# arhik/GaussianSplat

Hardware: AMD Instinct MI355X
Metric: fwd+bwd Msplats/sec at 1M Gaussians, 1920x1080, SH deg 3 (higher is better)
Workload: dtype f32; 1 GPU; C3: 1000000 gaussians, 1920x1080, SH3, ONE camera view per step, fwd+bwd; the steps cycle over the cameras [0, 4] (view k: eye rotated about +y by 45k degrees; one view slot per camera); synthetic scene of SURVEY 8d with the quaternions NORMALISED (8d leaves N(0,1)^4 raw: the reference never normalises q and |q| scales every footprint by |q|^4; un-normalised q is parity-tested, tests/test_gpu_size; views_per_rank=1, nranks=1, settle_steps=24, rank_mode=1, binning_rounds=1, schedule=3, view_slots=True, order=depth_desc, tile=16, instances=30150056, coarse_instances=2175944, walked_fwd=8350144, alpha_cull=True, list_cap=0, tile_parts=1, lists_capped=False

## Files before the change

gaussiansplat_amd/backend.py:

```python
from __future__ import annotations

import ctypes as C
import os

import numpy as np

_HERE = os.path.dirname(os.path.abspath(__file__))
LIB_PATH = os.environ.get("GSPLAT_HIP_LIB") or os.path.join(_HERE, "lib", "libgsplat_hip.so")

GS_MEM_HOST, GS_MEM_DEVICE = 0, 1
ORDER_INDEX, ORDER_DEPTH_DESC, ORDER_DEPTH_ASC = 0, 1, 2

(ARR_TS, ARR_TPS, ARR_MU, ARR_COV3D, ARR_COV2D, ARR_INVCOV, ARR_BBS, ARR_RGB, ARR_SIG, ARR_DEPTH_KEY,
 ARR_TILE_RECT, ARR_SORT_IDXS, ARR_TILE_RANGES, ARR_SORTED_IDS, ARR_SORTED_KEYS, ARR_GRAD2D) = range(16)

STAGES = ("preprocess", "depth_sort", "count_scan", "emit", "tile_sort", "ranges", "composite_fwd",
          "composite_bwd", "preprocess_bwd")

SYMBOLS = ("gs_default_config", "gs_abi_version", "gs_create", "gs_destroy", "gs_last_error", "gs_set_stream",
           "gs_synchronize", "gs_set_model", "gs_set_model_2d", "gs_set_image_size", "gs_set_camera", "gs_preprocess", "gs_bin", "gs_bind_outputs", "gs_forward", "gs_backward_sgd",
           "gs_backward", "gs_backward_ex", "gs_reset_grads", "gs_loss_l1_dssim", "gs_sgd_step", "gs_comm_unique_id",
           "gs_comm_init", "gs_allreduce_grads", "gs_comm_destroy", "gs_color_grads_pack", "gs_sh_grads_from_views", "gs_grads_alloc", "gs_grads_read", "gs_num_gaussians", "gs_num_instances", "gs_get_array",
           "gs_get_stage_times", "gs_get_stage_stats", "gs_get_work_counters", "gs_get_work_counters_ex", "gs_debug_time_composite",
           "gs_debug_tile_clock", "gs_debug_clock_mhz", "gs_rank_probe_result", "gs_num_rounds", "gs_set_view_slot", "gs_num_coarse_instances",
           "gs_get_list_stats", "gs_get_tile_parts", "gs_get_bin_path", "gs_debug_set_window", "gs_debug_tile_clock_rows", "gs_debug_tail_fill",
           "gs_adam_step", "gs_backward_adam")

GS_ABI_VERSION = 3
GS_DEBUG_WIDE_CURSORS = 1
GS_DEBUG_ALWAYS_ORDER = 2
GS_DEBUG_SUPER16 = 8
GS_DEBUG_SUPER8 = 16
GS_DEBUG_NO_TAIL_FILL = 32
GS_DEBUG_TINY_CAPS = 4
GS_MAX_VIEW_SLOTS = 4096
GS_ADAM_GROUPS = 6
GS_ADAM_SELECTIVE = 1
GS_ERR_INVALID, GS_ERR_UNSUPPORTED = -1, -5


class GsConfig(C.Structure):
    _fields_ = [("struct_size", C.c_int32), ("abi_version", C.c_int32), ("tile_size", C.c_int32), ("order", C.c_int32), ("t_min", C.c_float),
                ("deterministic", C.c_int32), ("export_debug", C.c_int32), ("profile_stages", C.c_int32),
                ("bin_path", C.c_int32), ("rank_mode", C.c_int32), ("alpha_cull", C.c_int32), ("schedule", C.c_int32),
                ("slab_mode", C.c_int32), ("slab_max_ratio", C.c_float), ("slab_fractions", C.c_float * 3), ("debug_flags", C.c_int32),
                ("depth_sort", C.c_int32), ("list_cap", C.c_int32), ("tile_parts", C.c_int32), ("reserved", C.c_int32 * 3)]


class GsGrads(C.Structure):
    _fields_ = [("d_means", C.c_void_p), ("d_scales", C.c_void_p), ("d_quats", C.c_void_p),
                ("d_opacities", C.c_void_p), ("d_shs", C.c_void_p)]


class GsError(RuntimeError):
    def __init__(self, code: int, msg: str):
        super().__init__(f"libgsplat_hip error {code}: {msg}")
# ... 397 lines not shown
```

gaussiansplat_amd/build.py:

```python
from __future__ import annotations

import os
import subprocess
import sys
from concurrent.futures import ThreadPoolExecutor

HERE = os.path.dirname(os.path.abspath(__file__))
CSRC = os.path.join(HERE, "csrc")
OUT_DIR = os.path.join(HERE, "lib")
LIB = os.path.join(OUT_DIR, "libgsplat_hip.so")
ARCH = "gfx950"

SOURCES = {
    "gs_preprocess.hip": ["-ffp-contract=off"],
    "gs_preprocess2d.hip": ["-ffp-contract=off"],
    "gs_preprocess_bwd.hip": [],
    "gs_sort.hip": [],
    "gs_bin2.hip": [],
    "gs_bin3.hip": [],
    "gs_bin_small.hip": [],
    "gs_composite.hip": ["-fno-slp-vectorize"],
    "gs_loss.hip": ["-fno-slp-vectorize"],
    "gs_adam.hip": ["-ffp-contract=off"],
    "gs_api.hip": [],
    "gs_api_bin.hip": [],
    "gs_api_composite.hip": [],
    "gs_api_comm.hip": [],
    "gs_api_debug.hip": [],
}
COMMON = ["-O3", "-fPIC", "-std=c++17", f"--offload-arch={ARCH}", "-Wall", "-Wno-unused-function"]


def _hipcc() -> str:
    for cand in (os.environ.get("HIPCC"), "/opt/rocm/bin/hipcc", "hipcc"):
        if cand and (os.path.isabs(cand) and os.path.exists(cand) or not os.path.isabs(cand)):
            return cand
    return "hipcc"


def _deps() -> float:
    hdrs = [os.path.join(CSRC, f) for f in os.listdir(CSRC) if f.endswith(".h")]
    hdrs.append(os.path.join(HERE, "..", "include", "gsplat.h"))
    return max(os.path.getmtime(h) for h in hdrs)


def build(force: bool = False, verbose: bool = False, tag: str = "", defines=()) -> str:
    out_dir = os.path.join(HERE, "lib_" + tag) if tag else OUT_DIR
    lib = os.path.join(out_dir, "libgsplat_hip.so")
    os.makedirs(out_dir, exist_ok=True)
    hipcc = _hipcc()
    hdr_time = _deps()
    objs, jobs = [], []
    for src, extra in SOURCES.items():
        extra = [*extra, *defines]
        s = os.path.join(CSRC, src)
        o = os.path.join(out_dir, src.replace(".hip", ".o"))
        objs.append(o)
        if force or not os.path.exists(o) or os.path.getmtime(o) < max(os.path.getmtime(s), hdr_time):
            jobs.append([hipcc, *COMMON, *extra, "-c", s, "-o", o])

    def run(cmd):
        if verbose:
            print(" ".join(cmd), flush=True)
        r = subprocess.run(cmd, capture_output=True, text=True)
# ... 17 lines not shown
```

gaussiansplat_amd/csrc/gs_api.hip:

```cpp
#include "gs_ctx.h"

std::string g_create_error;

extern "C" {

void gs_default_config(gs_config *cfg) {
    if (!cfg) return;
    std::memset(cfg, 0, sizeof(*cfg));
    cfg->struct_size = (int32_t)sizeof(gs_config);
    cfg->abi_version = GS_ABI_VERSION;
    cfg->tile_size = GS_TILE;
    cfg->order = GS_ORDER_DEPTH_DESC;
    cfg->t_min = 1e-5f;
    cfg->deterministic = 0;
    cfg->export_debug = 0;
    cfg->profile_stages = 0;
    cfg->rank_mode = 1;
    cfg->alpha_cull = 1;
    cfg->schedule = 3;
    cfg->slab_mode = 1;
}

int gs_abi_version(void) { return GS_ABI_VERSION; }

const char *gs_last_error(const gs_ctx *ctx) { return ctx ? ctx->err.c_str() : g_create_error.c_str(); }

int gs_create(gs_ctx **out, int device, const gs_config *cfg) {
    if (!out) return fail(nullptr, GS_ERR_INVALID, "gs_create: out is NULL");
    *out = nullptr;
    gs_config c0;
    gs_default_config(&c0);
    if (cfg) {
        if (cfg->struct_size != (int32_t)sizeof(gs_config) || cfg->abi_version != GS_ABI_VERSION)
            return fail(nullptr, GS_ERR_INVALID, "gs_create: gs_config.struct_size / abi_version mismatch (caller built against another gsplat.h)");
        c0 = *cfg;
    }
    if (c0.schedule == 0) c0.schedule = 3;
    if (c0.tile_size != GS_TILE) return fail(nullptr, GS_ERR_UNSUPPORTED, "gs_create: only tile_size 16 is supported (reference threads=(16,16))");
    if (c0.order < GS_ORDER_INDEX || c0.order > GS_ORDER_DEPTH_ASC) return fail(nullptr, GS_ERR_INVALID, "gs_create: bad order");
    if (!(c0.t_min >= 0.0f)) return fail(nullptr, GS_ERR_INVALID, "gs_create: t_min must be >= 0");
    if (c0.schedule != 1 && c0.schedule != 3 && c0.schedule != 4) return fail(nullptr, GS_ERR_INVALID, "gs_create: bad schedule (0, 1, 3 or 4)");
    if (c0.slab_mode < 0 || c0.slab_mode > 1) return fail(nullptr, GS_ERR_INVALID, "gs_create: bad slab_mode");
    if (c0.bin_path < 0 || c0.bin_path > 3) return fail(nullptr, GS_ERR_INVALID, "gs_create: bad bin_path");
    if (!(c0.slab_max_ratio >= 0.0f && c0.slab_max_ratio <= 1.0f)) return fail(nullptr, GS_ERR_INVALID, "gs_create: slab_max_ratio must be in [0, 1]");
    for (int i = 0; i < 3; ++i)
        if (!(c0.slab_fractions[i] >= 0.0f && c0.slab_fractions[i] < 1.0f)) return fail(nullptr, GS_ERR_INVALID, "gs_create: slab_fractions must be in [0, 1)");
    if (c0.debug_flags & ~(GS_DEBUG_WIDE_CURSORS | GS_DEBUG_ALWAYS_ORDER | GS_DEBUG_TINY_CAPS | GS_DEBUG_SUPER16 | GS_DEBUG_SUPER8 | GS_DEBUG_NO_TAIL_FILL)) return fail(nullptr, GS_ERR_INVALID, "gs_create: unknown debug_flags");
    if (c0.depth_sort < 0 || c0.depth_sort > 2) return fail(nullptr, GS_ERR_INVALID, "gs_create: depth_sort must be 0, 1 or 2");
    if (c0.list_cap < 0 || c0.list_cap > 2) return fail(nullptr, GS_ERR_INVALID, "gs_create: list_cap must be 0, 1 or 2");
    if (c0.tile_parts != 0 && c0.tile_parts != 1 && c0.tile_parts != 2 && c0.tile_parts != 4) return fail(nullptr, GS_ERR_INVALID, "gs_create: tile_parts must be 0, 1, 2 or 4");
    int ndev = 0;
    hipError_t e = hipGetDeviceCount(&ndev);
    if (e != hipSuccess || ndev <= 0)
        return fail(nullptr, GS_ERR_NO_DEVICE, "gs_create: no HIP device (this library has no CPU fallback)");
    if (device < 0 || device >= ndev) return fail(nullptr, GS_ERR_INVALID, "gs_create: device index out of range");
    gs_ctx *c = new (std::nothrow) gs_ctx();
    if (!c) return fail(nullptr, GS_ERR_OOM, "gs_create: host allocation failed");
    c->device = device;
    c->cfg = c0;
    c->slots.resize(GS_MAX_VIEW_SLOTS + 1);
    if ((e = hipSetDevice(device)) != hipSuccess) { delete c; return hipfail(nullptr, e, "hipSetDevice"); }
    if ((e = hipStreamCreateWithFlags(&c->stream, hipStreamNonBlocking)) != hipSuccess) { delete c; return hipfail(nullptr, e, "hipStreamCreate"); }
    c->own_stream = true;
    {
        hipDeviceProp_t prop;
        if (hipGetDeviceProperties(&prop, device) == hipSuccess && prop.multiProcessorCount > 0) c->wave_slots = prop.multiProcessorCount * 4 * 5;
        else (void)hipGetLastError();
    }
    if ((e = hipHostMalloc((void **)&c->pinned, sizeof(PinnedWords), hipHostMallocCoherent | hipHostMallocMapped)) != hipSuccess) { (void)hipStreamDestroy(c->stream); delete c; return hipfail(nullptr, e, "hipHostMalloc"); }
    if ((e = hipHostMalloc((void **)&c->pinned_split, sizeof(uint32_t) * 2 * (GS_MAX_VIEW_SLOTS + 1), hipHostMallocCoherent | hipHostMallocMapped)) != hipSuccess) {
// ... 315 lines not shown
```

gaussiansplat_amd/csrc/gs_api_composite.hip:

```cpp
#include "gs_ctx.h"

using Snap = gs_ctx::FramePlan::Snap;

static const uint32_t *forward_order(gs_ctx *c, const uint32_t **split) {
    const int64_t ntiles = (int64_t)c->gx * c->gy;
    if (!lpt_schedule(c) || ntiles <= 0 || ntiles > GS_LPT_MAX_TILES) return nullptr;
    const int k = order_index(c);
    if (k == GS_MAX_VIEW_SLOTS && c->cfg.schedule != 4) return nullptr;
    gs_ctx::ViewSlot &vs = c->slots[k];
    if (vs.tiles != c->grid_key()) return nullptr;
    if (c->order_pending) {
        if (hipStreamWaitEvent(c->stream, c->ev_order, 0) != hipSuccess) return nullptr;
        c->order_pending = false;
    }
    *split = c->split_word(k, vs.sel);
    return vs.order[vs.sel].as<uint32_t>();
}

static int parts_that_fit(const gs_ctx *c, int units) {
    const long long w = (long long)units * c->gx * c->gy;
    return 4 * w <= c->wave_slots ? 4 : 2 * w <= c->wave_slots ? 2 : 1;
}

static void plan_frame(gs_ctx *c, const uint32_t *order, const uint32_t *order_split, const uint32_t *hist) {
// ... 273 lines not shown
        GsPreprocess2DBwdArgs b2{};
        b2.n = c->n; b2.W = c->cam.W; b2.H = c->cam.H;
        b2.scales = c->scales; b2.rots = c->quats; b2.opac = c->opac;
        b2.g2d = det ? nullptr : c->g2d.as<float>(); b2.g2d_fixed = det ? c->g2d.as<long long>() : nullptr;
        b2.overwrite = (flags & GS_BWD_OVERWRITE) ? 1 : 0;
        b2.d_means = grads->d_means; b2.d_scales = grads->d_scales; b2.d_rots = grads->d_quats;
        b2.d_opac = grads->d_opacities; b2.d_colors = grads->d_shs;
        {
            StageTimer t(c, GS_STAGE_PREPROCESS_BWD);
            HIPCHK(c, gs_launch_preprocess2d_bwd(b2, c->stream));
        }
        if (mem == GS_MEM_HOST) HIPCHK(c, hipStreamSynchronize(c->stream));
        c->did_bwd = true;
        return GS_OK;
    }
    GsPreprocessBwdArgs b{};
    b.n = c->n; b.sh_degree = c->sh_degree;
    b.means = c->means; b.scales = c->scales; b.quats = c->quats; b.opac = c->opac; b.shs = c->shs;
    b.g2d = det ? nullptr : c->g2d.as<float>(); b.g2d_fixed = det ? c->g2d.as<long long>() : nullptr;
    HIPCHK(c, c->dpc.ensure(sizeof(float) * 4 * n1));
    b.dpc = c->dpc.as<float>();
    b.overwrite = (flags & GS_BWD_OVERWRITE) ? 1 : 0;
    b.shs_zeroed = fill_shs ? 1 : 0;
    b.sgd_scale = sgd_scale;
    b.d_means = grads->d_means; b.d_scales = grads->d_scales; b.d_quats = grads->d_quats;
    b.d_opac = grads->d_opacities; b.d_shs = grads->d_shs;
    {
        StageTimer t(c, GS_STAGE_PREPROCESS_BWD);
        HIPCHK(c, gs_launch_preprocess_bwd(b, c->cam, c->stream, chain ? chain : 3, adam, adam_mode));
    }
    if (mem == GS_MEM_HOST) HIPCHK(c, hipStreamSynchronize(c->stream));
    c->did_bwd = true;
    return GS_OK;
}

int gs_color_grads_pack(gs_ctx *c, float *drgb) {
    if (!c || !drgb) return GS_ERR_INVALID;
    if (c->kind != 0) return fail(c, GS_ERR_UNSUPPORTED, "gs_color_grads_pack: 3-D renderer only");
    if (!c->did_bwd) return fail(c, GS_ERR_INVALID, "gs_color_grads_pack: gs_backward first");
    if (bind_device(c)) return GS_ERR_HIP;
    const bool det = c->cfg.deterministic != 0;
    HIPCHK(c, gs_launch_pack_drgb(det ? nullptr : c->g2d.as<float>(), det ? c->g2d.as<long long>() : nullptr, drgb, c->n, c->stream));
    return GS_OK;
}

int gs_sh_grads_from_views(gs_ctx *c, int32_t nviews, const float *cams, const float *drgb, float *d_shs, int flags) {
// ... 13 lines not shown
```

gaussiansplat_amd/csrc/gs_common.h:

```cpp
#pragma once
#include <hip/hip_runtime.h>
#include <stdint.h>

#define GS_TILE 16
#define GS_WAVE 64

#define GS_PAYLOAD_QUADS 4
#define GS_BIG 1.0e30f
struct __attribute__((aligned(16))) GsPayload {
    float mx, my;
    float l2s;
    float xlo;
    float ka, kb, kc;
    float xhi;
    float r, g, b;
    float ylo;
    float yhi;
    float sig;
    uint32_t bbx;
    uint32_t bby;
};
static_assert(sizeof(GsPayload) == 16 * GS_PAYLOAD_QUADS, "payload row size");
__host__ __device__ inline void gs_payload_box_edges(GsPayload &p) {
    const int xmin = (int)(short)(p.bbx & 0xFFFFu), xmax = (int)(short)(p.bbx >> 16);
// ... 266 lines not shown
#endif
__host__ __device__ inline uint32_t gs_seg_len_all(uint32_t w, int seg_n) {
    if (GS_SEG_ALL_SHORT && w >= 80u && w <= (seg_n == 2 ? 192u : 64u * (uint32_t)seg_n + 64u)) return 64u;
    const uint32_t per = seg_n == 2 ? (w * GS_SEG_ALL_NUM + GS_SEG_ALL_DEN - 1u) / GS_SEG_ALL_DEN : (w + (uint32_t)seg_n - 1u) / (uint32_t)seg_n, sl = ((per + 63u) & ~63u) < (uint32_t)GS_SEG_ALL_MIN_LEN ? (uint32_t)GS_SEG_ALL_MIN_LEN : ((per + 63u) & ~63u);
    return w > sl ? sl : 0u;
}
int gs_seg_units(int front);
int gs_composite_grid_blocks(const GsCompositeArgs &a, int bwd);
hipError_t gs_launch_composite_fwd(const GsCompositeArgs &a, hipStream_t s);
hipError_t gs_launch_composite_bwd(const GsCompositeArgs &a, hipStream_t s);

#include "gs_adam.h"

struct GsPreprocessBwdArgs {
    int64_t n;
    int sh_degree;
    const float *means, *scales, *quats, *opac, *shs;
    const float *g2d;
    const long long *g2d_fixed;
    float *d_means, *d_scales, *d_quats, *d_opac, *d_shs;
    float *dpc;
    int overwrite;
    int shs_zeroed;
    float sgd_scale;
};
hipError_t gs_launch_preprocess_bwd(const GsPreprocessBwdArgs &a, const GsCamera &cam, hipStream_t s, int phases = 3,
                                    const GsAdamFused *adam = nullptr, int adam_mode = 0);

hipError_t gs_launch_pack_drgb(const float *g2d, const long long *g2d_fixed, float *out, int64_t n, hipStream_t s);
hipError_t gs_launch_sh_from_views(int64_t n, int sh_degree, const float *means, int nviews, const float *cams, const float *drgb,
                                   float *d_shs, int overwrite, hipStream_t s);

template <typename R>
__host__ __device__ inline void gs_g2d_to_grads(R (&g2)[10], R sig, R i0, R mc, R i3) {
#pragma clang fp contract(off)
    const R S0 = g2[3], Sx = g2[4], Sy = g2[5], Sxx = g2[6], Sxy = g2[7], Syy = g2[9];
    g2[3] = sig > R(0) ? -S0 / sig : R(0);
    g2[4] = -(i0 * Sx + mc * Sy);
    g2[5] = -(mc * Sx + i3 * Sy);
    g2[6] = R(0.5) * Sxx; g2[7] = R(0.5) * Sxy; g2[8] = R(0.5) * Sxy; g2[9] = R(0.5) * Syy;
}

#define GS_FIXED_SCALE 1099511627776.0f
#define GS_FIXED_INV (1.0 / 1099511627776.0)
#define GS_FIXED_SCALE2 268435456.0f
#define GS_FIXED_INV2 (1.0 / 268435456.0)
// ... 8 lines not shown
```

gaussiansplat_amd/csrc/gs_preprocess_bwd.hip:

```cpp
#include "gs_common.h"
#include <stdlib.h>

#ifndef GS_NT_STORES
#define GS_NT_STORES 2
#endif
#define SH_C0 0.28209479177387814f
#define SH_C1 0.48860251190291990f
__constant__ float bC2[5] = {1.0925484305920792f, -1.0925484305920792f, 0.31539156525252005f,
                             -1.0925484305920792f, 0.5462742152960396f};
__constant__ float bC3[7] = {-0.5900435899266435f, 2.890611442640554f, -0.4570457994644658f, 0.3731763325901154f,
                             -0.4570457994644658f, 1.445305721320277f, -0.5900435899266435f};

__device__ __forceinline__ void load_g2(const GsPreprocessBwdArgs &a, int64_t g, float (&o)[10]) {
    if (a.g2d_fixed) {
#pragma unroll
        for (int i = 0; i < 10; ++i) o[i] = (float)((double)a.g2d_fixed[GS_G2D_STRIDE * g + i] * gs_fixed_inv(i));
    } else {
        const float4 *r = reinterpret_cast<const float4 *>(a.g2d + GS_G2D_STRIDE * g);
        const float4 v0 = r[0], v1 = r[1], v2 = r[2];
        o[0] = v0.x; o[1] = v0.y; o[2] = v0.z; o[3] = v0.w; o[4] = v1.x; o[5] = v1.y; o[6] = v1.z; o[7] = v1.w; o[8] = v2.x; o[9] = v2.y;
    }
}

__device__ __forceinline__ float add_exact(float old, float v) {
// ... 7 lines not shown
template <int DEG, bool OVERWRITE, bool FUSED, int ADAM = 0>
__global__ __launch_bounds__(256) void gs_sh_bwd_kernel(GsPreprocessBwdArgs a, GsCamera cam, GsAdamFused ad) {
#pragma clang fp contract(off)
    constexpr int K = (DEG + 1) * (DEG + 1);
    constexpr int ROW = 3 * K + 1;
    extern __shared__ __attribute__((aligned(16))) float tile[];
    constexpr bool SKIP = !OVERWRITE;
    __shared__ uint8_t srow_live[256];
    const int64_t gb = (int64_t)blockIdx.x * blockDim.x;
    const int nb = (int)min((int64_t)blockDim.x, a.n - gb);
    float g2[10];
    if (SKIP) {
        const int64_t g0 = gb + threadIdx.x;
        bool lv = false;
        if (g0 < a.n) { load_g2(a, g0, g2); lv = g2[0] != 0.0f || g2[1] != 0.0f || g2[2] != 0.0f; }
        srow_live[threadIdx.x] = lv ? 1 : 0;
        __syncthreads();
    }
    constexpr bool VEC = (3 * K) % 4 == 0;
    const bool vec_out = VEC && (reinterpret_cast<uintptr_t>(a.d_shs) & 15) == 0;
    const int64_t g = gb + threadIdx.x;
    if (g < a.n) {
        if (!SKIP) load_g2(a, g, g2);
        const bool live = g2[0] != 0.0f || g2[1] != 0.0f || g2[2] != 0.0f;
        const float grgb[3] = {g2[0], g2[1], g2[2]};
        const float *T = cam.T, *P = cam.P;
        const float m1 = a.means[3 * g], m2 = a.means[3 * g + 1], m3 = a.means[3 * g + 2];
        float t[4], p[4];
#pragma unroll
        for (int i = 0; i < 4; ++i) t[i] = T[i] * m1 + T[i + 4] * m2 + T[i + 8] * m3 + T[i + 12];
#pragma unroll
        for (int i = 0; i < 4; ++i) p[i] = P[i] * t[0] + P[i + 4] * t[1] + P[i + 8] * t[2] + P[i + 12] * t[3];
        const float v0 = p[0] - (cam.lookAt[0] - cam.eye[0]);
        const float v1 = p[1] - (cam.lookAt[1] - cam.eye[1]);
        const float v2 = p[2] - (cam.lookAt[2] - cam.eye[2]);
        const float inrm = live ? rsqrtf(v0 * v0 + v1 * v1 + v2 * v2) : 0.0f;
        const float X = live ? v0 * inrm : 0.0f, Y = live ? v1 * inrm : 0.0f, Z = live ? v2 * inrm : 0.0f;
        float bs[K];
        bs[0] = SH_C0;
        if constexpr (DEG >= 1) { bs[1] = -Y * SH_C1; bs[2] = Z * SH_C1; bs[3] = -X * SH_C1; }
        if constexpr (DEG >= 2) {
            const float xx = X * X, yy = Y * Y, zz = Z * Z, xy = X * Y, yz = Y * Z, xz = X * Z;
            bs[4] = bC2[0] * xy; bs[5] = bC2[1] * yz; bs[6] = bC2[2] * (2 * zz - xx - yy); bs[7] = bC2[3] * xz; bs[8] = bC2[4] * (xx - yy);
            if constexpr (DEG >= 3) {
                bs[9] = bC3[0] * Y * (3 * xx - yy); bs[10] = bC3[1] * xy * Z; bs[11] = bC3[2] * Y * (4 * zz - xx - yy);
                bs[12] = bC3[3] * Z * (2 * zz - 3 * xx - 3 * yy); bs[13] = bC3[4] * X * (4 * zz - xx - yy);
                bs[14] = bC3[5] * Z * (xx - yy); bs[15] = bC3[6] * X * (xx - 3 * yy);
            }
        }
        float *sh = tile + threadIdx.x * ROW;
#pragma unroll
        for (int k = 0; k < K; ++k) {
#pragma unroll
            for (int c = 0; c < 3; ++c) sh[c + 3 * k] = bs[k] * grgb[c];
        }
        if (OVERWRITE && ADAM == 0) srow_live[threadIdx.x] = live ? 1 : 0;
        float ddir[3] = {0.0f, 0.0f, 0.0f};
        if (live) {
            const float4 *row = reinterpret_cast<const float4 *>(a.shs + (int64_t)3 * K * g);
            float shv[3 * K];
            if constexpr ((3 * K) % 4 == 0) {
#pragma unroll
                for (int q = 0; q < 3 * K / 4; ++q) { const float4 t4 = row[q]; shv[4 * q] = t4.x; shv[4 * q + 1] = t4.y; shv[4 * q + 2] = t4.z; shv[4 * q + 3] = t4.w; }
            } else {
#pragma unroll
                for (int q = 0; q < 3 * K; ++q) shv[q] = a.shs[(int64_t)3 * K * g + q];
            }
            float cs[K];
#pragma unroll
            for (int k = 0; k < K; ++k) cs[k] = grgb[0] * shv[3 * k] + grgb[1] * shv[3 * k + 1] + grgb[2] * shv[3 * k + 2];
            if constexpr (DEG >= 1) { ddir[0] += -SH_C1 * cs[3]; ddir[1] += -SH_C1 * cs[1]; ddir[2] += SH_C1 * cs[2]; }
            if constexpr (DEG >= 2) {
                ddir[0] += bC2[0] * Y * cs[4] - 2 * bC2[2] * X * cs[6] + bC2[3] * Z * cs[7] + 2 * bC2[4] * X * cs[8];
                ddir[1] += bC2[0] * X * cs[4] + bC2[1] * Z * cs[5] - 2 * bC2[2] * Y * cs[6] - 2 * bC2[4] * Y * cs[8];
                ddir[2] += bC2[1] * Y * cs[5] + 4 * bC2[2] * Z * cs[6] + bC2[3] * X * cs[7];
            }
            if constexpr (DEG >= 3) {
                const float xx = X * X, yy = Y * Y, zz = Z * Z, xy = X * Y, yz = Y * Z, xz = X * Z;
                ddir[0] += 6 * bC3[0] * xy * cs[9] + bC3[1] * yz * cs[10] - 2 * bC3[2] * xy * cs[11] - 6 * bC3[3] * xz * cs[12]
                           + bC3[4] * (4 * zz - 3 * xx - yy) * cs[13] + 2 * bC3[5] * xz * cs[14] + bC3[6] * (3 * xx - 3 * yy) * cs[15];
                ddir[1] += bC3[0] * (3 * xx - 3 * yy) * cs[9] + bC3[1] * xz * cs[10] + bC3[2] * (4 * zz - xx - 3 * yy) * cs[11]
                           - 6 * bC3[3] * yz * cs[12] - 2 * bC3[4] * xy * cs[13] - 2 * bC3[5] * yz * cs[14] - 6 * bC3[6] * xy * cs[15];
                ddir[2] += bC3[1] * xy * cs[10] + 8 * bC3[2] * yz * cs[11] + bC3[3] * (6 * zz - 3 * xx - 3 * yy) * cs[12]
                           + 8 * bC3[4] * xz * cs[13] + bC3[5] * (xx - yy) * cs[14];
            }
        }
        const float dd = X * ddir[0] + Y * ddir[1] + Z * ddir[2];
        const float4 dpc_sh = make_float4((ddir[0] - X * dd) * inrm, (ddir[1] - Y * dd) * inrm, (ddir[2] - Z * dd) * inrm, 0.0f);
        if (FUSED) {
            const float (&g2f)[10] = g2;
#define GS_GEOM_DPC dpc_sh
#define GS_GEOM_ADAM
            do {
#include "gs_geom_bwd_body.inc"
            } while (0);
#undef GS_GEOM_ADAM
#undef GS_GEOM_DPC
        } else reinterpret_cast<float4 *>(a.dpc)[g] = dpc_sh;
    }
    __syncthreads();
    if constexpr (ADAM != 0) {
        const int64_t o = gb * 3 * K;
        float *ps = const_cast<float *>(a.shs) + o, *ms = ad.m[4] + o, *vs = ad.v[4] + o;
        const bool vec = VEC && ((reinterpret_cast<uintptr_t>(a.shs) | reinterpret_cast<uintptr_t>(ad.m[4]) | reinterpret_cast<uintptr_t>(ad.v[4])) & 15) == 0;
        const float ss4 = ad.h.step_size[4], ss5 = ad.h.step_size[5];
        int nrow = nb;
        __shared__ int srow_order[ADAM == 2 ? 256 : 1], swave_live[16];
        if constexpr (ADAM == 2) {
            const int lane = threadIdx.x & 63, wv = threadIdx.x >> 6;
            const bool l = threadIdx.x < nb && srow_live[threadIdx.x];
            const unsigned long long b = __ballot(l);
// ... 42 lines not shown
                    const float4 o = dst[i4];
                    if (a.sgd_scale != 0.0f) { v.x = fmaf(a.sgd_scale, v.x, o.x); v.y = fmaf(a.sgd_scale, v.y, o.y); v.z = fmaf(a.sgd_scale, v.z, o.z); v.w = fmaf(a.sgd_scale, v.w, o.w); }
                    else { v.x += o.x; v.y += o.y; v.z += o.z; v.w += o.w; }
                }
                if (OVERWRITE && GS_NT_STORES) {
                    typedef float v4f __attribute__((ext_vector_type(4)));
                    const v4f vv = {v.x, v.y, v.z, v.w};
                    __builtin_nontemporal_store(vv, reinterpret_cast<v4f *>(dst) + i4);
                } else dst[i4] = v;
            }
        } else {
            for (int idx = threadIdx.x; idx < nb * 3 * K; idx += blockDim.x) {
                const bool lv = srow_live[idx / (3 * K)] != 0;
                if ((!OVERWRITE || a.shs_zeroed) && !lv) continue;
                const float v = (OVERWRITE && !lv) ? 0.0f : tile[(idx / (3 * K)) * ROW + idx % (3 * K)];
                if (OVERWRITE) a.d_shs[gb * 3 * K + idx] = v;
                else if (a.sgd_scale != 0.0f) a.d_shs[gb * 3 * K + idx] = fmaf(a.sgd_scale, v, a.d_shs[gb * 3 * K + idx]);
                else a.d_shs[gb * 3 * K + idx] += v;
            }
        }
    }
}

template <bool OVERWRITE>
__global__ __launch_bounds__(256) void gs_geom_bwd_kernel(GsPreprocessBwdArgs a, GsCamera cam) {
    const int64_t g = (int64_t)blockIdx.x * blockDim.x + threadIdx.x;
    if (g >= a.n) return;
    float g2f[10];
    load_g2(a, g, g2f);
#define GS_GEOM_DPC (reinterpret_cast<const float4 *>(a.dpc)[g])
    do {
#include "gs_geom_bwd_body.inc"
    } while (0);
#undef GS_GEOM_DPC
}

__global__ __launch_bounds__(256) void gs_pack_drgb_kernel(const float *__restrict__ g2d, const long long *__restrict__ g2d_fixed,
                                                            float *__restrict__ out, int64_t n) {
    const int64_t i = (int64_t)blockIdx.x * blockDim.x + threadIdx.x;
    if (i >= 3 * n) return;
    const int64_t g = i / 3; const int c = (int)(i - 3 * g);
    out[i] = g2d_fixed ? (float)((double)g2d_fixed[GS_G2D_STRIDE * g + c] * GS_FIXED_INV) : g2d[GS_G2D_STRIDE * g + c];
}

template <int DEG, bool OVERWRITE>
__global__ __launch_bounds__(256) void gs_sh_from_views_kernel(int64_t n, const float *__restrict__ means, int nviews,
// ... 64 lines not shown
    switch (sh_degree) {
        case 0: GS_SV(0); break;
        case 1: GS_SV(1); break;
        case 2: GS_SV(2); break;
        case 3: GS_SV(3); break;
        default: return hipErrorInvalidValue;
    }
#undef GS_SV
    return hipGetLastError();
}

#ifndef GS_SHBWD_THREADS
#define GS_SHBWD_THREADS 256
#endif
static int sh_bwd_threads() { return GS_SHBWD_THREADS; }
hipError_t gs_launch_preprocess_bwd(const GsPreprocessBwdArgs &a, const GsCamera &cam, hipStream_t s, int phases, const GsAdamFused *adam,
                                    int adam_mode) {
    if (a.n <= 0) return hipSuccess;
    const int T = sh_bwd_threads();
    dim3 block(T), grid((unsigned)((a.n + T - 1) / T));
    const int K = (a.sh_degree + 1) * (a.sh_degree + 1);
    const size_t lds = sizeof(float) * T * (3 * K + 1);
    const GsAdamFused ad = adam ? *adam : GsAdamFused{};
    if (adam_mode) {
        if (!adam || !a.overwrite || (phases & 3) != 3 || (adam_mode != 1 && adam_mode != 2)) return hipErrorInvalidValue;
#define GS_SHA(D) do { if (adam_mode == 2) hipLaunchKernelGGL((gs_sh_bwd_kernel<D, true, true, 2>), grid, block, lds, s, a, cam, ad); \
                       else hipLaunchKernelGGL((gs_sh_bwd_kernel<D, true, true, 1>), grid, block, lds, s, a, cam, ad); } while (0)
        switch (a.sh_degree) {
            case 0: GS_SHA(0); break;
            case 1: GS_SHA(1); break;
            case 2: GS_SHA(2); break;
            case 3: GS_SHA(3); break;
            default: return hipErrorInvalidValue;
        }
#undef GS_SHA
        return hipGetLastError();
    }
#define GS_SH2(D, F) do { if (a.overwrite) hipLaunchKernelGGL((gs_sh_bwd_kernel<D, true, F>), grid, block, lds, s, a, cam, ad); \
                         else hipLaunchKernelGGL((gs_sh_bwd_kernel<D, false, F>), grid, block, lds, s, a, cam, ad); } while (0)
#define GS_SH(D) do { if (fused) GS_SH2(D, true); else GS_SH2(D, false); } while (0)
    const bool fused = (phases & 3) == 3;
    if (phases & 1)
    switch (a.sh_degree) {
        case 0: GS_SH(0); break;
        case 1: GS_SH(1); break;
        case 2: GS_SH(2); break;
        case 3: GS_SH(3); break;
        default: return hipErrorInvalidValue;
    }
    block = dim3(256); grid = dim3((unsigned)((a.n + 255) / 256));
    if ((phases & 2) && !fused) {
        if (a.overwrite) hipLaunchKernelGGL(gs_geom_bwd_kernel<true>, grid, block, 0, s, a, cam);
        else hipLaunchKernelGGL(gs_geom_bwd_kernel<false>, grid, block, 0, s, a, cam);
    }
    return hipGetLastError();
}
```

include/gsplat.h:

```cpp
#ifndef GSPLAT_H
#define GSPLAT_H

#include <stdint.h>

#ifdef __cplusplus
extern "C" {
#endif

#define GS_ABI_VERSION 3

typedef enum {
    GS_OK = 0,
    GS_ERR_INVALID = -1,
    GS_ERR_NO_DEVICE = -2,
    GS_ERR_HIP = -3,
    GS_ERR_OOM = -4,
    GS_ERR_UNSUPPORTED = -5
} gs_status;

typedef enum { GS_MEM_HOST = 0, GS_MEM_DEVICE = 1 } gs_mem;

typedef enum { GS_ORDER_INDEX = 0, GS_ORDER_DEPTH_DESC = 1, GS_ORDER_DEPTH_ASC = 2 } gs_order;

typedef struct {
// ... 4 lines not shown
    float   t_min;
    int32_t deterministic;
    int32_t export_debug;
    int32_t profile_stages;
    int32_t bin_path;
    int32_t rank_mode;
    int32_t alpha_cull;
    int32_t schedule;
    int32_t slab_mode;
    float   slab_max_ratio;
    float   slab_fractions[3];
    int32_t debug_flags;
    int32_t depth_sort;
    int32_t list_cap;
    int32_t tile_parts;
    int32_t reserved[3];
} gs_config;
#define GS_DEBUG_WIDE_CURSORS 1
#define GS_DEBUG_ALWAYS_ORDER 2
#define GS_DEBUG_SUPER16 8
#define GS_DEBUG_SUPER8 16
#define GS_DEBUG_TINY_CAPS 4
#define GS_DEBUG_NO_TAIL_FILL 32

typedef struct gs_ctx gs_ctx;

void gs_default_config(gs_config *cfg);

int gs_abi_version(void);

int gs_create(gs_ctx **out, int device, const gs_config *cfg);
int gs_destroy(gs_ctx *ctx);
const char *gs_last_error(const gs_ctx *ctx);

#define GS_STREAM_LEGACY ((void *)1)
int gs_set_stream(gs_ctx *ctx, void *hip_stream);
int gs_synchronize(gs_ctx *ctx);

int gs_set_model(gs_ctx *ctx, int64_t n, int sh_degree,
                 const float *means, const float *scales, const float *quats,
                 const float *opacities, const float *shs, int mem);

int gs_set_model_2d(gs_ctx *ctx, int64_t n, const float *means, const float *scales, const float *rotations,
                    const float *opacities, const float *colors, int mem);
int gs_set_image_size(gs_ctx *ctx, int32_t W, int32_t H);

// ... 127 lines not shown
```

Baseline: 839.1 Msplats/s.

## Compact live Gaussians per block in fused preprocess backward kernel

Adds a new fused SH+geometry backward kernel that first loads each Gaussian's 2D gradients, ballots which rows are live, and compacts the live indices into a shared list. The heavy SH and geometry backward math then runs only on the compacted live rows, so wavefronts are not occupied by culled Gaussians. Dead rows are zero-filled separately when overwriting. This costs an extra g2 reload and more shared memory and control logic, and adds a debug flag to fall back to the old kernel.

```diff
diff --git a/gaussiansplat_amd/backend.py b/gaussiansplat_amd/backend.py
--- a/gaussiansplat_amd/backend.py
+++ b/gaussiansplat_amd/backend.py
@@ -32,6 +32,7 @@
 GS_DEBUG_SUPER16 = 8
 GS_DEBUG_SUPER8 = 16
 GS_DEBUG_NO_TAIL_FILL = 32
+GS_DEBUG_NO_LIVE_COMPACT = 64
 GS_DEBUG_TINY_CAPS = 4
 GS_MAX_VIEW_SLOTS = 4096
 GS_ADAM_GROUPS = 6
diff --git a/gaussiansplat_amd/build.py b/gaussiansplat_amd/build.py
--- a/gaussiansplat_amd/build.py
+++ b/gaussiansplat_amd/build.py
@@ -39,7 +39,7 @@
 
 
 def _deps() -> float:
-    hdrs = [os.path.join(CSRC, f) for f in os.listdir(CSRC) if f.endswith(".h")]
+    hdrs = [os.path.join(CSRC, f) for f in os.listdir(CSRC) if f.endswith((".h", ".inc"))]
     hdrs.append(os.path.join(HERE, "..", "include", "gsplat.h"))
     return max(os.path.getmtime(h) for h in hdrs)
 
diff --git a/gaussiansplat_amd/csrc/gs_api.hip b/gaussiansplat_amd/csrc/gs_api.hip
--- a/gaussiansplat_amd/csrc/gs_api.hip
+++ b/gaussiansplat_amd/csrc/gs_api.hip
@@ -45,7 +45,7 @@
     if (!(c0.slab_max_ratio >= 0.0f && c0.slab_max_ratio <= 1.0f)) return fail(nullptr, GS_ERR_INVALID, "gs_create: slab_max_ratio must be in [0, 1]");
     for (int i = 0; i < 3; ++i)
         if (!(c0.slab_fractions[i] >= 0.0f && c0.slab_fractions[i] < 1.0f)) return fail(nullptr, GS_ERR_INVALID, "gs_create: slab_fractions must be in [0, 1)");
-    if (c0.debug_flags & ~(GS_DEBUG_WIDE_CURSORS | GS_DEBUG_ALWAYS_ORDER | GS_DEBUG_TINY_CAPS | GS_DEBUG_SUPER16 | GS_DEBUG_SUPER8 | GS_DEBUG_NO_TAIL_FILL)) return fail(nullptr, GS_ERR_INVALID, "gs_create: unknown debug_flags");
+    if (c0.debug_flags & ~(GS_DEBUG_WIDE_CURSORS | GS_DEBUG_ALWAYS_ORDER | GS_DEBUG_TINY_CAPS | GS_DEBUG_SUPER16 | GS_DEBUG_SUPER8 | GS_DEBUG_NO_TAIL_FILL | GS_DEBUG_NO_LIVE_COMPACT)) return fail(nullptr, GS_ERR_INVALID, "gs_create: unknown debug_flags");
     if (c0.depth_sort < 0 || c0.depth_sort > 2) return fail(nullptr, GS_ERR_INVALID, "gs_create: depth_sort must be 0, 1 or 2");
     if (c0.list_cap < 0 || c0.list_cap > 2) return fail(nullptr, GS_ERR_INVALID, "gs_create: list_cap must be 0, 1 or 2");
     if (c0.tile_parts != 0 && c0.tile_parts != 1 && c0.tile_parts != 2 && c0.tile_parts != 4) return fail(nullptr, GS_ERR_INVALID, "gs_create: tile_parts must be 0, 1, 2 or 4");
diff --git a/gaussiansplat_amd/csrc/gs_api_composite.hip b/gaussiansplat_amd/csrc/gs_api_composite.hip
--- a/gaussiansplat_amd/csrc/gs_api_composite.hip
+++ b/gaussiansplat_amd/csrc/gs_api_composite.hip
@@ -319,6 +319,7 @@
     b.dpc = c->dpc.as<float>();
     b.overwrite = (flags & GS_BWD_OVERWRITE) ? 1 : 0;
     b.shs_zeroed = fill_shs ? 1 : 0;
+    b.no_live_compact = (c->cfg.debug_flags & GS_DEBUG_NO_LIVE_COMPACT) ? 1 : 0;
     b.sgd_scale = sgd_scale;
     b.d_means = grads->d_means; b.d_scales = grads->d_scales; b.d_quats = grads->d_quats;
     b.d_opac = grads->d_opacities; b.d_shs = grads->d_shs;
diff --git a/gaussiansplat_amd/csrc/gs_common.h b/gaussiansplat_amd/csrc/gs_common.h
--- a/gaussiansplat_amd/csrc/gs_common.h
+++ b/gaussiansplat_amd/csrc/gs_common.h
@@ -312,6 +312,7 @@
     float *dpc;
     int overwrite;
     int shs_zeroed;
+    int no_live_compact;
     float sgd_scale;
 };
 hipError_t gs_launch_preprocess_bwd(const GsPreprocessBwdArgs &a, const GsCamera &cam, hipStream_t s, int phases = 3,
diff --git a/gaussiansplat_amd/csrc/gs_preprocess_bwd.hip b/gaussiansplat_amd/csrc/gs_preprocess_bwd.hip
--- a/gaussiansplat_amd/csrc/gs_preprocess_bwd.hip
+++ b/gaussiansplat_amd/csrc/gs_preprocess_bwd.hip
@@ -53,71 +53,9 @@
     const int64_t g = gb + threadIdx.x;
     if (g < a.n) {
         if (!SKIP) load_g2(a, g, g2);
-        const bool live = g2[0] != 0.0f || g2[1] != 0.0f || g2[2] != 0.0f;
-        const float grgb[3] = {g2[0], g2[1], g2[2]};
-        const float *T = cam.T, *P = cam.P;
-        const float m1 = a.means[3 * g], m2 = a.means[3 * g + 1], m3 = a.means[3 * g + 2];
-        float t[4], p[4];
-#pragma unroll
-        for (int i = 0; i < 4; ++i) t[i] = T[i] * m1 + T[i + 4] * m2 + T[i + 8] * m3 + T[i + 12];
-#pragma unroll
-        for (int i = 0; i < 4; ++i) p[i] = P[i] * t[0] + P[i + 4] * t[1] + P[i + 8] * t[2] + P[i + 12] * t[3];
-        const float v0 = p[0] - (cam.lookAt[0] - cam.eye[0]);
-        const float v1 = p[1] - (cam.lookAt[1] - cam.eye[1]);
-        const float v2 = p[2] - (cam.lookAt[2] - cam.eye[2]);
-        const float inrm = live ? rsqrtf(v0 * v0 + v1 * v1 + v2 * v2) : 0.0f;
-        const float X = live ? v0 * inrm : 0.0f, Y = live ? v1 * inrm : 0.0f, Z = live ? v2 * inrm : 0.0f;
-        float bs[K];
-        bs[0] = SH_C0;
-        if constexpr (DEG >= 1) { bs[1] = -Y * SH_C1; bs[2] = Z * SH_C1; bs[3] = -X * SH_C1; }
-        if constexpr (DEG >= 2) {
-            const float xx = X * X, yy = Y * Y, zz = Z * Z, xy = X * Y, yz = Y * Z, xz = X * Z;
-            bs[4] = bC2[0] * xy; bs[5] = bC2[1] * yz; bs[6] = bC2[2] * (2 * zz - xx - yy); bs[7] = bC2[3] * xz; bs[8] = bC2[4] * (xx - yy);
-            if constexpr (DEG >= 3) {
-                bs[9] = bC3[0] * Y * (3 * xx - yy); bs[10] = bC3[1] * xy * Z; bs[11] = bC3[2] * Y * (4 * zz - xx - yy);
-                bs[12] = bC3[3] * Z * (2 * zz - 3 * xx - 3 * yy); bs[13] = bC3[4] * X * (4 * zz - xx - yy);
-                bs[14] = bC3[5] * Z * (xx - yy); bs[15] = bC3[6] * X * (xx - 3 * yy);
-            }
-        }
         float *sh = tile + threadIdx.x * ROW;
-#pragma unroll
-        for (int k = 0; k < K; ++k) {
-#pragma unroll
-            for (int c = 0; c < 3; ++c) sh[c + 3 * k] = bs[k] * grgb[c];
-        }
+#include "gs_sh_bwd_part.inc"
         if (OVERWRITE && ADAM == 0) srow_live[threadIdx.x] = live ? 1 : 0;
-        float ddir[3] = {0.0f, 0.0f, 0.0f};
-        if (live) {
-            const float4 *row = reinterpret_cast<const float4 *>(a.shs + (int64_t)3 * K * g);
-            float shv[3 * K];
-            if constexpr ((3 * K) % 4 == 0) {
-#pragma unroll
-                for (int q = 0; q < 3 * K / 4; ++q) { const float4 t4 = row[q]; shv[4 * q] = t4.x; shv[4 * q + 1] = t4.y; shv[4 * q + 2] = t4.z; shv[4 * q + 3] = t4.w; }
-            } else {
-#pragma unroll
-                for (int q = 0; q < 3 * K; ++q) shv[q] = a.shs[(int64_t)3 * K * g + q];
-            }
-            float cs[K];
-#pragma unroll
-            for (int k = 0; k < K; ++k) cs[k] = grgb[0] * shv[3 * k] + grgb[1] * shv[3 * k + 1] + grgb[2] * shv[3 * k + 2];
-            if constexpr (DEG >= 1) { ddir[0] += -SH_C1 * cs[3]; ddir[1] += -SH_C1 * cs[1]; ddir[2] += SH_C1 * cs[2]; }
-            if constexpr (DEG >= 2) {
-                ddir[0] += bC2[0] * Y * cs[4] - 2 * bC2[2] * X * cs[6] + bC2[3] * Z * cs[7] + 2 * bC2[4] * X * cs[8];
-                ddir[1] += bC2[0] * X * cs[4] + bC2[1] * Z * cs[5] - 2 * bC2[2] * Y * cs[6] - 2 * bC2[4] * Y * cs[8];
-                ddir[2] += bC2[1] * Y * cs[5] + 4 * bC2[2] * Z * cs[6] + bC2[3] * X * cs[7];
-            }
-            if constexpr (DEG >= 3) {
-                const float xx = X * X, yy = Y * Y, zz = Z * Z, xy = X * Y, yz = Y * Z, xz = X * Z;
-                ddir[0] += 6 * bC3[0] * xy * cs[9] + bC3[1] * yz * cs[10] - 2 * bC3[2] * xy * cs[11] - 6 * bC3[3] * xz * cs[12]
-                           + bC3[4] * (4 * zz - 3 * xx - yy) * cs[13] + 2 * bC3[5] * xz * cs[14] + bC3[6] * (3 * xx - 3 * yy) * cs[15];
-                ddir[1] += bC3[0] * (3 * xx - 3 * yy) * cs[9] + bC3[1] * xz * cs[10] + bC3[2] * (4 * zz - xx - 3 * yy) * cs[11]
-                           - 6 * bC3[3] * yz * cs[12] - 2 * bC3[4] * xy * cs[13] - 2 * bC3[5] * yz * cs[14] - 6 * bC3[6] * xy * cs[15];
-                ddir[2] += bC3[1] * xy * cs[10] + 8 * bC3[2] * yz * cs[11] + bC3[3] * (6 * zz - 3 * xx - 3 * yy) * cs[12]
-                           + 8 * bC3[4] * xz * cs[13] + bC3[5] * (xx - yy) * cs[14];
-            }
-        }
-        const float dd = X * ddir[0] + Y * ddir[1] + Z * ddir[2];
-        const float4 dpc_sh = make_float4((ddir[0] - X * dd) * inrm, (ddir[1] - Y * dd) * inrm, (ddir[2] - Z * dd) * inrm, 0.0f);
         if (FUSED) {
             const float (&g2f)[10] = g2;
 #define GS_GEOM_DPC dpc_sh
@@ -206,6 +144,181 @@
     }
 }
 
+#ifndef GS_LIVE_GB
+#define GS_LIVE_GB 256
+#endif
+static_assert(GS_LIVE_GB % 256 == 0 && GS_LIVE_GB >= 256 && GS_LIVE_GB <= 1024, "GS_LIVE_GB: 256, 512, 768 or 1024");
+
+template <int DEG, bool OVERWRITE, int ADAM = 0>
+__global__ __launch_bounds__(256) void gs_live_bwd_kernel(GsPreprocessBwdArgs a, GsCamera cam, GsAdamFused ad) {
+#pragma clang fp contract(off)
+    constexpr int K = (DEG + 1) * (DEG + 1);
+    constexpr int ROW = 3 * K + 1;
+    constexpr int GB = GS_LIVE_GB, NQ = GB / 256;
+    constexpr bool VEC = (3 * K) % 4 == 0;
+    extern __shared__ __attribute__((aligned(16))) float tile[];
+    __shared__ uint16_t slist[GB];
+    __shared__ uint8_t sblk_live[GB];
+    __shared__ uint8_t srow_live[256];
+    __shared__ int scnt[NQ * 4];
+    const int64_t gb = (int64_t)blockIdx.x * GB;
+    const int nb = (int)min((int64_t)GB, a.n - gb);
+    const int lane = threadIdx.x & 63, wv = threadIdx.x >> 6;
+    float g2[10];
+    bool lv[NQ];
+    unsigned long long bal[NQ];
+#pragma unroll
+    for (int q = 0; q < NQ; ++q) {
+        const int row = q * 256 + (int)threadIdx.x;
+        lv[q] = false;
+        if (row < nb) {
+            load_g2(a, gb + row, g2);
+#pragma unroll
+            for (int i = 0; i < 10; ++i) lv[q] = lv[q] || g2[i] != 0.0f;
+        }
+        bal[q] = __ballot(lv[q]);
+        if (lane == 0) scnt[q * 4 + wv] = __popcll(bal[q]);
+        sblk_live[row] = lv[q] ? 1 : 0;
+    }
+    __syncthreads();
+    int nlive = 0;
+    {
+        int before[NQ];
+#pragma unroll
+        for (int q = 0; q < NQ; ++q) {
+            before[q] = 0;
+#pragma unroll
+            for (int w = 0; w < 4; ++w) { const int c = scnt[q * 4 + w]; if (w == wv) before[q] = nlive; nlive += c; }
+        }
+#pragma unroll
+        for (int q = 0; q < NQ; ++q)
+            if (lv[q]) slist[before[q] + __popcll(bal[q] & ((1ull << lane) - 1ull))] = (uint16_t)(q * 256 + (int)threadIdx.x);
+    }
+    if constexpr (OVERWRITE && ADAM == 0) {
+        if (nlive < nb && blockIdx.y == 0) {
+            for (int idx = threadIdx.x; idx < 3 * nb; idx += 256) {
+                if (sblk_live[idx / 3]) continue;
+                if (a.d_means) { if (GS_NT_STORES > 1) __builtin_nontemporal_store(0.0f, &a.d_means[3 * gb + idx]); else a.d_means[3 * gb + idx] = 0.0f; }
+                if (a.d_scales) { if (GS_NT_STORES > 1) __builtin_nontemporal_store(0.0f, &a.d_scales[3 * gb + idx]); else a.d_scales[3 * gb + idx] = 0.0f; }
+            }
+            for (int row = threadIdx.x; row < nb; row += 256) {
+                if (sblk_live[row]) continue;
+                if (a.d_quats) reinterpret_cast<float4 *>(a.d_quats)[gb + row] = make_float4(0.f, 0.f, 0.f, 0.f);
+                if (a.d_opac) { if (GS_NT_STORES > 1) __builtin_nontemporal_store(0.0f, &a.d_opac[gb + row]); else a.d_opac[gb + row] = 0.0f; }
+            }
+            if (a.d_shs && !a.shs_zeroed) {
+                if (VEC && (reinterpret_cast<uintptr_t>(a.d_shs) & 15) == 0) {
+                    float4 *dst = reinterpret_cast<float4 *>(a.d_shs + gb * 3 * K);
+                    for (int i4 = threadIdx.x; i4 < nb * (3 * K / 4); i4 += 256) {
+                        if (sblk_live[(i4 * 4) / (3 * K)]) continue;
+                        if (GS_NT_STORES) {
+                            typedef float v4f __attribute__((ext_vector_type(4)));
+                            const v4f z = {0.0f, 0.0f, 0.0f, 0.0f};
+                            __builtin_nontemporal_store(z, reinterpret_cast<v4f *>(dst) + i4);
+                        } else dst[i4] = make_float4(0.f, 0.f, 0.f, 0.f);
+                    }
+                } else {
+                    for (int idx = threadIdx.x; idx < nb * 3 * K; idx += 256)
+                        if (!sblk_live[idx / (3 * K)]) a.d_shs[gb * 3 * K + idx] = 0.0f;
+                }
+            }
+        }
+    }
+    const int r0 = 256 * (int)blockIdx.y;
+    if (r0 >= nlive) return;
+    __syncthreads();
+    {
+        const int cnt = min(256, nlive - r0);
+        if ((int)threadIdx.x < cnt) {
+            const int64_t g = gb + slist[r0 + threadIdx.x];
+            load_g2(a, g, g2);
+            float *sh = tile + threadIdx.x * ROW;
+#include "gs_sh_bwd_part.inc"
+            if (ADAM == 0) srow_live[threadIdx.x] = live ? 1 : 0;
+            const float (&g2f)[10] = g2;
+#define GS_GEOM_DPC dpc_sh
+#define GS_GEOM_ADAM
+            do {
+#include "gs_geom_bwd_body.inc"
+            } while (0);
+#undef GS_GEOM_ADAM
+#undef GS_GEOM_DPC
+        }
+        __syncthreads();
+        if constexpr (ADAM != 0) {
+            float *ps = const_cast<float *>(a.shs), *ms = ad.m[4], *vs = ad.v[4];
+            const bool vec = VEC && ((reinterpret_cast<uintptr_t>(ps) | reinterpret_cast<uintptr_t>(ms) | reinterpret_cast<uintptr_t>(vs)) & 15) == 0;
+            const float ss4 = ad.h.step_size[4], ss5 = ad.h.step_size[5];
+            __shared__ uint8_t srow_order[256];
+            __shared__ int swave_live[4];
+            const bool l = (int)threadIdx.x < cnt && srow_live[threadIdx.x];
+            const unsigned long long b = __ballot(l);
+            if (lane == 0) swave_live[wv] = __popcll(b);
+            __syncthreads();
+            int off = 0, nrow = 0;
+            for (int w = 0; w < 4; ++w) { off += w < wv ? swave_live[w] : 0; nrow += swave_live[w]; }
+            if (l) srow_order[off + __popcll(b & ((1ull << lane) - 1ull))] = (uint8_t)threadIdx.x;
+            __syncthreads();
+            if (vec) {
+                for (int c4 = threadIdx.x; c4 < nrow * (3 * K / 4); c4 += 256) {
+                    const int ri = (c4 * 4) / (3 * K), j = (c4 * 4) % (3 * K);
+                    const int row = srow_order[ri];
+                    const int64_t i4 = ((gb + slist[r0 + row]) * 3 * K + j) / 4;
+                    const float *t = tile + row * ROW + j;
+                    float4 p = reinterpret_cast<float4 *>(ps)[i4], m = reinterpret_cast<float4 *>(ms)[i4], v = reinterpret_cast<float4 *>(vs)[i4];
+                    gs_adam_update(p.x, m.x, v.x, t[0], ad.h, j < 3 ? ss4 : ss5);
+                    gs_adam_update(p.y, m.y, v.y, t[1], ad.h, j + 1 < 3 ? ss4 : ss5);
+                    gs_adam_update(p.z, m.z, v.z, t[2], ad.h, j + 2 < 3 ? ss4 : ss5);
+                    gs_adam_update(p.w, m.w, v.w, t[3], ad.h, j + 3 < 3 ? ss4 : ss5);
+                    reinterpret_cast<float4 *>(ps)[i4] = p; reinterpret_cast<float4 *>(ms)[i4] = m; reinterpret_cast<float4 *>(vs)[i4] = v;
+                }
+            } else {
+                for (int c = threadIdx.x; c < nrow * 3 * K; c += 256) {
+                    const int ri = c / (3 * K), j = c % (3 * K);
+                    const int row = srow_order[ri];
+                    const int64_t idx = (gb + slist[r0 + row]) * 3 * K + j;
+                    float p = ps[idx], m = ms[idx], v = vs[idx];
+                    gs_adam_update(p, m, v, tile[row * ROW + j], ad.h, j < 3 ? ss4 : ss5);
+                    ps[idx] = p; ms[idx] = m; vs[idx] = v;
+                }
+            }
+        } else if (a.d_shs) {
+            if (VEC && (reinterpret_cast<uintptr_t>(a.d_shs) & 15) == 0) {
+                for (int c4 = threadIdx.x; c4 < cnt * (3 * K / 4); c4 += 256) {
+                    const int row = (c4 * 4) / (3 * K), j = (c4 * 4) % (3 * K);
+                    const bool lvr = srow_live[row] != 0;
+                    if ((!OVERWRITE || a.shs_zeroed) && !lvr) continue;
+                    float4 *dst = reinterpret_cast<float4 *>(a.d_shs + (gb + slist[r0 + row]) * 3 * K + j);
+                    const float *t = tile + row * ROW + j;
+                    float4 v = make_float4(t[0], t[1], t[2], t[3]);
+                    if (OVERWRITE && !lvr) v = make_float4(0.0f, 0.0f, 0.0f, 0.0f);
+                    if (!OVERWRITE) {
+                        const float4 o = *dst;
+                        if (a.sgd_scale != 0.0f) { v.x = fmaf(a.sgd_scale, v.x, o.x); v.y = fmaf(a.sgd_scale, v.y, o.y); v.z = fmaf(a.sgd_scale, v.z, o.z); v.w = fmaf(a.sgd_scale, v.w, o.w); }
+                        else { v.x += o.x; v.y += o.y; v.z += o.z; v.w += o.w; }
+                    }
+                    if (OVERWRITE && GS_NT_STORES) {
+                        typedef float v4f __attribute__((ext_vector_type(4)));
+                        const v4f vv = {v.x, v.y, v.z, v.w};
+                        __builtin_nontemporal_store(vv, reinterpret_cast<v4f *>(dst));
+                    } else *dst = v;
+                }
+            } else {
+                for (int c = threadIdx.x; c < cnt * 3 * K; c += 256) {
+                    const int row = c / (3 * K), j = c % (3 * K);
+                    const bool lvr = srow_live[row] != 0;
+                    if ((!OVERWRITE || a.shs_zeroed) && !lvr) continue;
+                    float *dst = a.d_shs + (gb + slist[r0 + row]) * 3 * K + j;
+                    const float v = (OVERWRITE && !lvr) ? 0.0f : tile[row * ROW + j];
+                    if (OVERWRITE) *dst = v;
+                    else if (a.sgd_scale != 0.0f) *dst = fmaf(a.sgd_scale, v, *dst);
+                    else *dst += v;
+                }
+            }
+        }
+    }
+}
+
 template <bool OVERWRITE>
 __global__ __launch_bounds__(256) void gs_geom_bwd_kernel(GsPreprocessBwdArgs a, GsCamera cam) {
     const int64_t g = (int64_t)blockIdx.x * blockDim.x + threadIdx.x;
@@ -316,9 +429,13 @@
     const int K = (a.sh_degree + 1) * (a.sh_degree + 1);
     const size_t lds = sizeof(float) * T * (3 * K + 1);
     const GsAdamFused ad = adam ? *adam : GsAdamFused{};
+    const bool compact = !a.no_live_compact;
+    const dim3 lblock(256), lgrid((unsigned)((a.n + GS_LIVE_GB - 1) / GS_LIVE_GB), GS_LIVE_GB / 256);
+    const size_t llds = sizeof(float) * 256 * (3 * K + 1);
     if (adam_mode) {
         if (!adam || !a.overwrite || (phases & 3) != 3 || (adam_mode != 1 && adam_mode != 2)) return hipErrorInvalidValue;
-#define GS_SHA(D) do { if (adam_mode == 2) hipLaunchKernelGGL((gs_sh_bwd_kernel<D, true, true, 2>), grid, block, lds, s, a, cam, ad); \
+#define GS_SHA(D) do { if (adam_mode == 2 && compact) hipLaunchKernelGGL((gs_live_bwd_kernel<D, true, 2>), lgrid, lblock, llds, s, a, cam, ad); \
+                       else if (adam_mode == 2) hipLaunchKernelGGL((gs_sh_bwd_kernel<D, true, true, 2>), grid, block, lds, s, a, cam, ad); \
                        else hipLaunchKernelGGL((gs_sh_bwd_kernel<D, true, true, 1>), grid, block, lds, s, a, cam, ad); } while (0)
         switch (a.sh_degree) {
             case 0: GS_SHA(0); break;
@@ -332,7 +449,9 @@
     }
 #define GS_SH2(D, F) do { if (a.overwrite) hipLaunchKernelGGL((gs_sh_bwd_kernel<D, true, F>), grid, block, lds, s, a, cam, ad); \
                          else hipLaunchKernelGGL((gs_sh_bwd_kernel<D, false, F>), grid, block, lds, s, a, cam, ad); } while (0)
-#define GS_SH(D) do { if (fused) GS_SH2(D, true); else GS_SH2(D, false); } while (0)
+#define GS_LV(D) do { if (a.overwrite) hipLaunchKernelGGL((gs_live_bwd_kernel<D, true>), lgrid, lblock, llds, s, a, cam, ad); \
+                      else hipLaunchKernelGGL((gs_live_bwd_kernel<D, false>), lgrid, lblock, llds, s, a, cam, ad); } while (0)
+#define GS_SH(D) do { if (fused && compact) GS_LV(D); else if (fused) GS_SH2(D, true); else GS_SH2(D, false); } while (0)
     const bool fused = (phases & 3) == 3;
     if (phases & 1)
     switch (a.sh_degree) {
diff --git a/gaussiansplat_amd/csrc/gs_sh_bwd_part.inc b/gaussiansplat_amd/csrc/gs_sh_bwd_part.inc
--- /dev/null
+++ b/gaussiansplat_amd/csrc/gs_sh_bwd_part.inc
@@ -0,0 +1,63 @@
+    const bool live = g2[0] != 0.0f || g2[1] != 0.0f || g2[2] != 0.0f;
+    const float grgb[3] = {g2[0], g2[1], g2[2]};
+    const float *T = cam.T, *P = cam.P;
+    const float m1 = a.means[3 * g], m2 = a.means[3 * g + 1], m3 = a.means[3 * g + 2];
+    float t[4], p[4];
+#pragma unroll
+    for (int i = 0; i < 4; ++i) t[i] = T[i] * m1 + T[i + 4] * m2 + T[i + 8] * m3 + T[i + 12];
+#pragma unroll
+    for (int i = 0; i < 4; ++i) p[i] = P[i] * t[0] + P[i + 4] * t[1] + P[i + 8] * t[2] + P[i + 12] * t[3];
+    const float v0 = p[0] - (cam.lookAt[0] - cam.eye[0]);
+    const float v1 = p[1] - (cam.lookAt[1] - cam.eye[1]);
+    const float v2 = p[2] - (cam.lookAt[2] - cam.eye[2]);
+    const float inrm = live ? rsqrtf(v0 * v0 + v1 * v1 + v2 * v2) : 0.0f;
+    const float X = live ? v0 * inrm : 0.0f, Y = live ? v1 * inrm : 0.0f, Z = live ? v2 * inrm : 0.0f;
+    float bs[K];
+    bs[0] = SH_C0;
+    if constexpr (DEG >= 1) { bs[1] = -Y * SH_C1; bs[2] = Z * SH_C1; bs[3] = -X * SH_C1; }
+    if constexpr (DEG >= 2) {
+        const float xx = X * X, yy = Y * Y, zz = Z * Z, xy = X * Y, yz = Y * Z, xz = X * Z;
+        bs[4] = bC2[0] * xy; bs[5] = bC2[1] * yz; bs[6] = bC2[2] * (2 * zz - xx - yy); bs[7] = bC2[3] * xz; bs[8] = bC2[4] * (xx - yy);
+        if constexpr (DEG >= 3) {
+            bs[9] = bC3[0] * Y * (3 * xx - yy); bs[10] = bC3[1] * xy * Z; bs[11] = bC3[2] * Y * (4 * zz - xx - yy);
+            bs[12] = bC3[3] * Z * (2 * zz - 3 * xx - 3 * yy); bs[13] = bC3[4] * X * (4 * zz - xx - yy);
+            bs[14] = bC3[5] * Z * (xx - yy); bs[15] = bC3[6] * X * (xx - 3 * yy);
+        }
+    }
+#pragma unroll
+    for (int k = 0; k < K; ++k) {
+#pragma unroll
+        for (int c = 0; c < 3; ++c) sh[c + 3 * k] = bs[k] * grgb[c];
+    }
+    float ddir[3] = {0.0f, 0.0f, 0.0f};
+    if (live) {
+        const float4 *row = reinterpret_cast<const float4 *>(a.shs + (int64_t)3 * K * g);
+        float shv[3 * K];
+        if constexpr ((3 * K) % 4 == 0) {
+#pragma unroll
+            for (int q = 0; q < 3 * K / 4; ++q) { const float4 t4 = row[q]; shv[4 * q] = t4.x; shv[4 * q + 1] = t4.y; shv[4 * q + 2] = t4.z; shv[4 * q + 3] = t4.w; }
+        } else {
+#pragma unroll
+            for (int q = 0; q < 3 * K; ++q) shv[q] = a.shs[(int64_t)3 * K * g + q];
+        }
+        float cs[K];
+#pragma unroll
+        for (int k = 0; k < K; ++k) cs[k] = grgb[0] * shv[3 * k] + grgb[1] * shv[3 * k + 1] + grgb[2] * shv[3 * k + 2];
+        if constexpr (DEG >= 1) { ddir[0] += -SH_C1 * cs[3]; ddir[1] += -SH_C1 * cs[1]; ddir[2] += SH_C1 * cs[2]; }
+        if constexpr (DEG >= 2) {
+            ddir[0] += bC2[0] * Y * cs[4] - 2 * bC2[2] * X * cs[6] + bC2[3] * Z * cs[7] + 2 * bC2[4] * X * cs[8];
+            ddir[1] += bC2[0] * X * cs[4] + bC2[1] * Z * cs[5] - 2 * bC2[2] * Y * cs[6] - 2 * bC2[4] * Y * cs[8];
+            ddir[2] += bC2[1] * Y * cs[5] + 4 * bC2[2] * Z * cs[6] + bC2[3] * X * cs[7];
+        }
+        if constexpr (DEG >= 3) {
+            const float xx = X * X, yy = Y * Y, zz = Z * Z, xy = X * Y, yz = Y * Z, xz = X * Z;
+            ddir[0] += 6 * bC3[0] * xy * cs[9] + bC3[1] * yz * cs[10] - 2 * bC3[2] * xy * cs[11] - 6 * bC3[3] * xz * cs[12]
+                       + bC3[4] * (4 * zz - 3 * xx - yy) * cs[13] + 2 * bC3[5] * xz * cs[14] + bC3[6] * (3 * xx - 3 * yy) * cs[15];
+            ddir[1] += bC3[0] * (3 * xx - 3 * yy) * cs[9] + bC3[1] * xz * cs[10] + bC3[2] * (4 * zz - xx - 3 * yy) * cs[11]
+                       - 6 * bC3[3] * yz * cs[12] - 2 * bC3[4] * xy * cs[13] - 2 * bC3[5] * yz * cs[14] - 6 * bC3[6] * xy * cs[15];
+            ddir[2] += bC3[1] * xy * cs[10] + 8 * bC3[2] * yz * cs[11] + bC3[3] * (6 * zz - 3 * xx - 3 * yy) * cs[12]
+                       + 8 * bC3[4] * xz * cs[13] + bC3[5] * (xx - yy) * cs[14];
+        }
+    }
+    const float dd = X * ddir[0] + Y * ddir[1] + Z * ddir[2];
+    const float4 dpc_sh = make_float4((ddir[0] - X * dd) * inrm, (ddir[1] - Y * dd) * inrm, (ddir[2] - Z * dd) * inrm, 0.0f);
diff --git a/include/gsplat.h b/include/gsplat.h
--- a/include/gsplat.h
+++ b/include/gsplat.h
@@ -50,6 +50,7 @@
 #define GS_DEBUG_SUPER8 16
 #define GS_DEBUG_TINY_CAPS 4
 #define GS_DEBUG_NO_TAIL_FILL 32
+#define GS_DEBUG_NO_LIVE_COMPACT 64
 
 typedef struct gs_ctx gs_ctx;
 
```

Measured after the change: 827.6 Msplats/s. -1.4%, worse.
